# yukiteruono/pbsim3

Measured on NVIDIA B200. Metric: simulated Gbp/s, higher is better.
Workload: dtype int32

## Files before the change

### pbsim_b200/csrc/engine.cu

```cuda
#include <cuda_runtime.h>

#include <algorithm>
#include <climits>
#include <cmath>
#include <cstdarg>
#include <cstdio>
#include <cstring>
#include <cub/device/device_radix_sort.cuh>
#include <cub/device/device_scan.cuh>
#include <condition_variable>
#include <deque>
#include <mutex>
#include <string>
#include <thread>
#include <vector>

#include "../../include/pbsim_cuda.h"
#include "emit.cuh"
#include "gz_kernels.cuh"
#include "k0_genome.cuh"
#include "model_image.hpp"
#include "sample_plan.hpp"
#include "seg_kernels.cuh"
#include "sim_kernels.cuh"
// ... 571 lines not shown
  const int64_t d0 = e->run.replay_starts[s0];
  const int64_t d1 = (s0 + n_sub < e->run.replay_nsubreads) ? e->run.replay_starts[s0 + n_sub] : e->run.replay_ndraws;
  c.next_start_after = (s0 + n_sub < e->run.replay_nsubreads) ? d1 : e->run.replay_ndraws;
  if (d0 < 0 || d1 < d0 || d1 > e->run.replay_ndraws) return fail(e, PBSIM_E_REPLAY, "replay starts are not monotone");
  if (upload(e, e->d_draws, e->run.replay_draws + d0, (size_t)(d1 - d0))) return PBSIM_E_CUDA;
  if (upload(e, e->d_starts, e->run.replay_starts + s0, (size_t)n_sub)) return PBSIM_E_CUDA;
  c.A.rng.draws = e->d_draws.as<int32_t>();
  c.A.rng.draws_base = d0;
  c.A.rng.draws_end = d1;
  c.A.rng.starts = e->d_starts.as<int64_t>();
  return 0;
}

int plan(pbsim_engine *e, BatchCtx &c) {
  Batch &B = e->B;
  const uint32_t seg_min_len = c.use_segments ? (uint32_t)e->seg_min_len : 0u;
  if (c.sample)
    k_plan_sample<<<nblk(B.n_reads, 256), 256, 0, e->st>>>(c.A.G, c.Pl, *c.sb, B, e->cap_num, e->cap_den, c.spec ? 1u : 0u,
                                                             c.A.rng.seed, c.A.M.uniform_bias ? 1u : 0u, seg_min_len);
  else
    k_plan<<<nblk(B.n_reads, 256), 256, 0, e->st>>>(c.A.M, c.A.G, device_set(e), c.A.rng, B, c.clip_room, e->cap_num,
                                                      e->cap_den, c.qs ? 8u : 16u, seg_min_len, e->seg_extra,
                                                      e->chain_chunk_eff());
  e->launches++;
  return schedule_ctas(e, e->d_bins, B.key_in, B.key_out, B.idx_in, B.order, B.n_sub, 0, c.cta_threads, true, &c.cta);
}

int size_slots(pbsim_engine *e, BatchCtx &c) {
  Batch &B = e->B;
  unsigned long long *hctrl = host_ctrl(e);
  unsigned long long *tmp = u64_slice(e, kSliceScanIn);
  unsigned long long *seg_off = u64_slice(e, kSliceSegOff), *chunk_off = u64_slice(e, kSliceChunkOff);
  int rc;
  if ((rc = widen_scan(e, B.cap, B.n_sub, tmp, reinterpret_cast<unsigned long long *>(B.ev_off)))) return rc;
  if ((rc = widen_scan(e, B.ck_cap, B.n_sub, tmp, reinterpret_cast<unsigned long long *>(B.ck_off)))) return rc;
  if (c.use_segments) {
    if ((rc = widen_scan(e, B.nseg, B.n_sub, tmp, seg_off))) return rc;
    if (peek(e, hctrl + 2, seg_off + B.n_sub, 8)) return PBSIM_E_CUDA;
    if ((rc = widen_scan(e, B.nchunk, B.n_sub, tmp, chunk_off))) return rc;
    if (peek(e, hctrl + 4, chunk_off + B.n_sub, 8)) return PBSIM_E_CUDA;
  }
  if (peek(e, hctrl, B.ev_off + B.n_sub, 8)) return PBSIM_E_CUDA;
  if (peek(e, hctrl + 1, B.ck_off + B.n_sub, 8)) return PBSIM_E_CUDA;
  CK(cudaStreamSynchronize(e->st));
  c.n_seg_total = c.use_segments ? hctrl[2] : 0;
  c.n_chunk_total = c.use_segments ? hctrl[4] : 0;
  if (c.n_seg_total > 0x7FFFFFF0ull) return fail(e, PBSIM_E_INVALID, "too many segments in one batch");
  CK(e->d_ev.ensure((size_t)hctrl[0] * (c.qs ? 2 : 1) + 256));
  CK(e->d_ck.ensure((size_t)hctrl[1] * sizeof(Ckpt) + 256));
  if (c.n_seg_total > 0) CK(e->d_seg.ensure((size_t)c.n_seg_total * (6 * 4 + sizeof(SegResult)) + 256));
  return 0;
}

void pass1_sequential(pbsim_engine *e, BatchCtx &c) {
  SimArgs &A = c.A;
  set_ctas(A, c.cta);
  A.ev = e->d_ev.as<uint8_t>();
  A.ck = e->d_ck.as<Ckpt>();
  const uint32_t grid = c.cta.slots;
  if (c.sample) {
    if (c.replay) k_sim_sample<PBSIM_RNG_REPLAY><<<grid, kSimThreads, 0, e->st>>>(A, c.Pl, *c.sb, 0u);
    else k_sim_sample<PBSIM_RNG_PHILOX><<<grid, kSimThreads, 0, e->st>>>(A, c.Pl, *c.sb, 0u);
  } else if (c.qs) {
    if (c.replay) k_sim_qshmm<PBSIM_RNG_REPLAY><<<grid, kSimThreads, kQsSmemBytes, e->st>>>(A);
    else k_sim_qshmm<PBSIM_RNG_PHILOX><<<grid, kSimThreads, kQsSmemBytes, e->st>>>(A);
  } else {
    const uint32_t smem = e->er_smem_bar_off + 16;
    if (c.replay) k_sim_errhmm<PBSIM_RNG_REPLAY><<<grid, kErrThreads, smem, e->st>>>(A, e->er_smem_bar_off);
    else k_sim_errhmm<PBSIM_RNG_PHILOX><<<grid, kErrThreads, smem, e->st>>>(A, e->er_smem_bar_off);
  }
  e->launches++;
}

int pass1_segments(pbsim_engine *e, BatchCtx &c) {
  const Batch &B = e->B;
  const uint32_t nseg = (uint32_t)c.n_seg_total;
  SegBatch S;
  S.n_seg_total = nseg;
  S.seg_off = reinterpret_cast<const uint64_t *>(u64_slice(e, kSliceSegOff));
  S.seg_res = e->d_seg.as<SegResult>();
  uint32_t *u = reinterpret_cast<uint32_t *>(S.seg_res + nseg);
  uint32_t **seg_arrays[] = {&S.seg_sub, &S.seg_key_in, &S.seg_key_out, &S.seg_id_in, &S.seg_order, &S.seg_state};
  for (size_t i = 0; i < 6; ++i) *seg_arrays[i] = u + i * nseg;
  k_seg_fill<<<nblk(B.n_sub, 256), 256, 0, e->st>>>(B, S, c.pass);
  CtaSchedule sc;
  int rc = schedule_ctas(e, e->d_seg_bins, S.seg_key_in, S.seg_key_out, S.seg_id_in, S.seg_order, nseg, 20, c.cta_threads,
                         false, &sc);
  if (rc) return rc;
  SegArgs SA;
  SA.keys = c.A.keys;
  SA.M = c.A.M;
  SA.G = c.A.G;
  SA.bias_one = e->d_biasone.as<uint8_t>();
  SA.B = B;
  SA.S = S;
  set_ctas(SA, sc);
  SA.ev = e->d_ev.as<uint8_t>();
  SA.pool_q = c.Pl.quals;
  SA.pool_start = c.Pl.start;
  if (c.n_chunk_total > 0) {
    const uint32_t nch = (uint32_t)c.n_chunk_total;
    const uint32_t chain_threads = c.qs ? (uint32_t)kChainThreads : c.cta_threads;
    CK(e->d_chunk.ensure((size_t)nch * 5 * 4 + 64));
    ChunkBatch C;
    C.n_chunks = nch;
    C.per_chunk = e->chain_chunk_eff();
    C.qs = c.qs ? 1u : 0u;
    C.chunk_off = reinterpret_cast<const uint64_t *>(u64_slice(e, kSliceChunkOff));
    uint32_t **chunk_arrays[] = {&C.sub, &C.key_in, &C.key_out, &C.id_in, &C.order};
    for (size_t i = 0; i < 5; ++i) *chunk_arrays[i] = e->d_chunk.as<uint32_t>() + i * nch;
    k_chunk_fill<<<nblk(B.n_sub, 256), 256, 0, e->st>>>(B, C, c.pass);
    CtaSchedule cc;
    if ((rc = schedule_ctas(e, e->d_chunk_bins, C.key_in, C.key_out, C.id_in, C.order, nch, 0, chain_threads, true, &cc)))
      return rc;
    SegArgs CA = SA;
    set_ctas(CA, cc);
    CK(cudaEventRecord(e->ev_chain[0], e->st));
    if (c.qs) k_chain_chunk<<<cc.slots, kChainThreads, kQsSmemBytes, e->st>>>(CA, C);
    else k_chain_chunk_err<<<cc.slots, kErrThreads, e->er_smem_bar_off + 16, e->st>>>(CA, C, e->er_smem_bar_off);
    CK(cudaEventRecord(e->ev_chain[1], e->st));
    e->launches += 2;
  }
  CK(cudaEventRecord(e->ev_seg[0], e->st));
  const uint32_t end_grid = nblk((uint64_t)B.n_sub * 32, 128);
  if (c.qs) {
    if (c.sample) k_sim_seg<true><<<sc.slots, kSimThreads, 0, e->st>>>(SA);
    else k_sim_seg<false><<<sc.slots, kSimThreads, 0, e->st>>>(SA);
    CK(cudaEventRecord(e->ev_seg[1], e->st));
    k_find_end<<<end_grid, 128, 0, e->st>>>(B, S, c.A.G, SA.bias_one, c.pass, SA.ev, e->d_ck.as<Ckpt>(), c.A.M.qs_fast,
                                            c.sample ? 1u : 0u);
  } else {
    k_sim_seg_err<<<sc.slots, kErrThreads, e->er_smem_bar_off + 16, e->st>>>(SA, e->er_smem_bar_off);
    CK(cudaEventRecord(e->ev_seg[1], e->st));
    k_find_end_err<<<end_grid, 128, 0, e->st>>>(B, S, c.A.G, SA.keys, SA.bias_one, c.pass, SA.ev, e->d_ck.as<Ckpt>());
  }
  e->launches += 3;
  e->seg_batches++;
  return 0;
}

int sample_redo(pbsim_engine *e, BatchCtx &c) {
  Batch &B = e->B;
  unsigned long long *ctrl = e->d_ctrl.as<unsigned long long>(), *hctrl = host_ctrl(e);
  hctrl[6] = 0;
  CK(cudaMemsetAsync(ctrl + 6, 0, 8, e->st));
  k_sample_redo<<<nblk(B.n_reads, 256), 256, 0, e->st>>>(B, ctrl + 6);
  if (peek(e, hctrl + 6, ctrl + 6, 8)) return PBSIM_E_CUDA;
  CK(cudaStreamSynchronize(e->st));
  e->launches += 2;
  if (hctrl[6] == 0) return 0;
  const int rc =
      schedule_ctas(e, e->d_bins, B.key_in, B.key_out, B.idx_in, B.order, B.n_sub, 0, c.cta_threads, true, &c.cta);
  if (rc) return rc;
  if (c.replay) k_sim_sample<PBSIM_RNG_REPLAY><<<c.cta.slots, kSimThreads, 0, e->st>>>(c.A, c.Pl, *c.sb, 1u);
  else k_sim_sample<PBSIM_RNG_PHILOX><<<c.cta.slots, kSimThreads, 0, e->st>>>(c.A, c.Pl, *c.sb, 1u);
  e->launches++;
  e->sample_redo_groups += (int64_t)hctrl[6];
  if (hctrl[6] * 2 > c.sb->n_groups) e->sample_spec_run = false;
  return 0;
}

int quota_cut(pbsim_engine *e, BatchCtx &c, int attempt) {
  const Batch &B = e->B;
  const uint32_t n_reads = B.n_reads, n_sub = B.n_sub;
  unsigned long long *ctrl = e->d_ctrl.as<unsigned long long>(), *hctrl = host_ctrl(e);
  unsigned long long *rl0 = u64_slice(e, kSliceScanIn);
  unsigned long long *prefix = u64_slice(e, kSliceRlen0Prefix);
  k_rlen0<<<nblk(n_reads, 256), 256, 0, e->st>>>(B.rlen, n_reads, c.pass, rl0);
  const int rc = excl_scan(e, rl0, prefix, n_reads);
  if (rc) return rc;
  hctrl[0] = n_reads;
  hctrl[1] = 0;
  hctrl[2] = 0;
  hctrl[3] = 0;
  CK(cudaMemcpyAsync(ctrl, hctrl, 32, cudaMemcpyHostToDevice, e->st));
  if (c.sample)
    k_find_cut_sample<<<nblk(n_reads, 256), 256, 0, e->st>>>(prefix, n_reads, e->len_total, e->run.len_quota, ctrl);
  else if (c.clip_room < 0)
    k_find_cut<<<nblk(n_reads, 256), 256, 0, e->st>>>(prefix, B.plan_raw, n_reads, e->len_total, e->run.len_quota, ctrl);
  k_batch_totals<<<nblk(n_sub, 256), 256, 0, e->st>>>(prefix, B.rlen, B.flags, n_reads, c.pass, ctrl);
  e->launches += 3;
  if (c.replay) {
    k_check_replay<<<nblk(n_sub, 256), 256, 0, e->st>>>(c.A.rng.starts, B.draws_used, B.plan_wlen, (uint32_t)e->glen, n_sub,
                                                        c.pass, c.next_start_after, ctrl,
                                                        reinterpret_cast<unsigned int *>(&ctrl[3]));
    e->launches++;
  }
  if (peek(e, hctrl, ctrl, 32)) return PBSIM_E_CUDA;
  CK(cudaStreamSynchronize(e->st));
  const uint32_t flags = (uint32_t)hctrl[2];
  if (flags & 2u) return fail(e, PBSIM_E_PARAM, "a read drew an accuracy for which the model has no usable tables");
  float pass1_ms = 0, ms = 0;
  CK(cudaEventElapsedTime(&pass1_ms, e->ev_k[0], e->ev_k[1]));
  e->sim_ms += pass1_ms;
  if (c.n_seg_total > 0) {
    CK(cudaEventElapsedTime(&ms, e->ev_seg[0], e->ev_seg[1]));
    e->seg_ms += ms;
    if (c.n_chunk_total > 0) {
      CK(cudaEventElapsedTime(&ms, e->ev_chain[0], e->ev_chain[1]));
      e->chain_ms += ms;
    }
  }
  if (getenv("PBSIM_DEBUG"))
    fprintf(stderr, "[pbsim] batch reads=%u sub=%u segments=%llu flags=%u pass1_ms=%.2f attempt=%d\n", n_reads, n_sub,
            (unsigned long long)c.n_seg_total, flags, pass1_ms, attempt);
  return 0;
}

int emit_batch(pbsim_engine *e, const BatchCtx &c, BatchResult *out) {
  const Batch &B = e->B;
  const uint32_t nv_sub = out->n_valid_reads * c.pass;
  if (nv_sub == 0) return 0;
  unsigned long long *hctrl = host_ctrl(e);

  unsigned long long *reads_size = u64_slice(e, kSliceReadsSize);
  unsigned long long *maf_size = u64_slice(e, kSliceMafSize);
  unsigned long long *ntiles = u64_slice(e, kSliceNtiles);
  unsigned long long *reads_off = u64_slice(e, kSliceReadsOff);
  unsigned long long *maf_off = u64_slice(e, kSliceMafOff);
// ... 551 lines not shown
  if (rc != 1) return rc;
  e->held_set = it.set;
  c->first_read = it.first_read;
  c->n_reads = it.n_reads;
  c->bases = it.bases;
  c->reads_bytes = (int64_t)it.reads_bytes;
  c->maf_bytes = (int64_t)it.maf_bytes;
  c->reads_text_bytes = (int64_t)it.reads_text_bytes;
  c->maf_text_bytes = (int64_t)it.maf_text_bytes;
  c->reads = reinterpret_cast<const char *>(e->out[it.set].reads.p);
  c->maf = reinterpret_cast<const char *>(e->out[it.set].maf.p);
  c->on_device = 1;
  return 1;
}

int build_replay_read_map(pbsim_engine *e) {
  const pbsim_run &run = e->run;
  const int64_t pass = e->model.pass_num;
  const int64_t n_logged = run.replay_nsubreads / pass;
  std::vector<uint32_t> map_tr, map_k;
  map_tr.reserve((size_t)n_logged);
  map_k.reserve((size_t)n_logged);
  int64_t idx = 0;
  for (uint32_t t = 0; t < (uint32_t)e->set_n && idx < n_logged; ++t) {
    const uint32_t tlen = e->h_set_start[t + 1] - e->h_set_start[t];
    const uint32_t rank = (tlen + 999u) / 1000u;
    for (uint64_t k = 1; k <= e->h_set_nr[t] && idx < n_logged; ++k) {
      const int64_t st = run.replay_starts[idx * pass];
      if (st < 0 || st + 3 > run.replay_ndraws) return fail(e, PBSIM_E_REPLAY, "replay log exhausted while mapping the reads of the set");
      const uint32_t d0 = (uint32_t)run.replay_draws[st], d1 = (uint32_t)run.replay_draws[st + 1],
                     d2 = (uint32_t)run.replay_draws[st + 2];
      uint32_t len = (uint32_t)e->h_prob2len[d0 % (uint32_t)e->model.len_rand_value];
      const uint32_t acc = e->h_prob2acc[d1 % (uint32_t)e->model.accuracy_rand_value];
      const uint32_t index = d2 % e->h_ssp_mod[rank] + 1u;
      uint32_t ssp = 100u;
      for (uint32_t j = 0; j < 21u; ++j) {
        const uint32_t en = e->h_ssp_ends[rank * 21u + j];
        if (en == 0xFFFFu) break;
        if (index <= en) {
          ssp = j * 5u;
          break;
        }
      }
      const double value = ssp == 0u ? 0.0 : ((double)ssp - 2.5) / 100;
      volatile double prod = (double)tlen * value;
      const uint32_t offset = (uint32_t)(int)(prod + 0.5);
      if ((uint64_t)offset + len > tlen) len = offset < tlen ? tlen - offset : 0u;
      map_tr.push_back(t);
      map_k.push_back((uint32_t)k);
      ++idx;
      if (acc == 100u) k = len;
    }
  }
  if (idx != n_logged)
    return fail(e, PBSIM_E_REPLAY, "the replay log holds %lld reads but the set accounts for %lld", (long long)n_logged,
                (long long)idx);
  int rc;
  if ((rc = upload(e, e->d_map_tr, map_tr.data(), map_tr.size()))) return rc;
  if ((rc = upload(e, e->d_map_k, map_k.data(), map_k.size()))) return rc;
  CK(cudaStreamSynchronize(e->st));
  e->replay_map = true;
  e->run.max_reads = idx;
  return 0;
}

}

extern "C" {

int pbsim_cuda_abi_version(void) { return PBSIM_ABI_VERSION; }

const char *pbsim_cuda_last_error(const pbsim_engine *e) { return e ? e->err.c_str() : g_create_error.c_str(); }

int pbsim_cuda_create(pbsim_engine **out, int device) {
  pbsim_engine *e = nullptr;
  if (!out) return fail(e, PBSIM_E_INVALID, "null output pointer");
  int n = 0;
  cudaError_t ce = cudaGetDeviceCount(&n);
  if (ce != cudaSuccess || n == 0)
    return fail(e, PBSIM_E_CUDA, "no usable CUDA device (%s); libpbsim_cuda has no CPU fallback",
                ce == cudaSuccess ? "device count is 0" : cudaGetErrorString(ce));
  if (device < 0 || device >= n) return fail(e, PBSIM_E_INVALID, "device %d out of range (0..%d)", device, n - 1);
  CK(cudaSetDevice(device));
  CK(cudaFuncSetAttribute(k_chain_chunk, cudaFuncAttributePreferredSharedMemoryCarveout, cudaSharedmemCarveoutMaxShared));
  CK(cudaFuncSetAttribute(k_emit_rows<PBSIM_METHOD_QSHMM>, cudaFuncAttributePreferredSharedMemoryCarveout,
                          cudaSharedmemCarveoutMaxShared));
  CK(cudaFuncSetAttribute(k_emit_rows<PBSIM_METHOD_ERRHMM>, cudaFuncAttributePreferredSharedMemoryCarveout,
                          cudaSharedmemCarveoutMaxShared));
  CK(cudaFuncSetAttribute(k_gz_encode, cudaFuncAttributeMaxDynamicSharedMemorySize, (int)kGzEncodeSmem));
  pbsim_engine *ne = new pbsim_engine();
  ne->device = device;
  cudaError_t c1 = cudaStreamCreateWithFlags(&ne->st, cudaStreamNonBlocking);
  cudaError_t c2 = cudaStreamCreateWithFlags(&ne->st_copy, cudaStreamNonBlocking);
  cudaError_t c3 = cudaEventCreate(&ne->ev0);
  cudaError_t c4 = cudaEventCreate(&ne->ev1);
  if (c1 != cudaSuccess || c2 != cudaSuccess || c3 != cudaSuccess || c4 != cudaSuccess) {
    delete ne;
    return fail(e, PBSIM_E_CUDA, "cannot create CUDA streams/events");
  }
  cudaEventCreate(&ne->ev_copy);
  for (auto &ev : ne->ev_k) cudaEventCreate(&ev);
  for (auto &ev : ne->ev_user) cudaEventCreate(&ev);
  for (auto &ev : ne->ev_gz) cudaEventCreate(&ev);
  for (auto &ev : ne->ev_seg) cudaEventCreate(&ev);
  for (auto &ev : ne->ev_chain) cudaEventCreate(&ev);
  std::memset(&ne->model, 0, sizeof ne->model);
  std::memset(&ne->emitp, 0, sizeof ne->emitp);
  *out = ne;
  return 0;
}

void pbsim_cuda_destroy(pbsim_engine *e) {
  if (!e) return;
  cudaSetDevice(e->device);
  stop_producer(e);
  cudaStreamSynchronize(e->st_copy);
  cudaStreamSynchronize(e->st);
  cudaEventDestroy(e->ev_copy);
  for (auto &ev : e->ev_k) cudaEventDestroy(ev);
  for (auto &ev : e->ev_user) cudaEventDestroy(ev);
  for (auto &ev : e->ev_gz) cudaEventDestroy(ev);
  for (auto &ev : e->ev_seg) cudaEventDestroy(ev);
  for (auto &ev : e->ev_chain) cudaEventDestroy(ev);
  cudaEventDestroy(e->ev0);
  cudaEventDestroy(e->ev1);
  cudaStreamDestroy(e->st);
  cudaStreamDestroy(e->st_copy);
  delete e;
}

int pbsim_cuda_set_model(pbsim_engine *e, const pbsim_model *m) {
  if (!e || !m) return PBSIM_E_INVALID;
  CK(cudaSetDevice(e->device));
  const bool sample = m->method == PBSIM_METHOD_SAMPLE;
  if (m->method != PBSIM_METHOD_QSHMM && m->method != PBSIM_METHOD_ERRHMM && !sample)
    return fail(e, PBSIM_E_INVALID, "method must be qshmm, errhmm or sample");
  if (sample && m->pass_num != 1)
    return fail(e, PBSIM_E_INVALID, "sampling-based simulation supports only single-pass");
  if (!sample &&
      (m->pass_num < 1 || m->len_rand_value < 1 || m->accuracy_rand_value < 1 || !m->prob2len || !m->prob2accuracy))
    return fail(e, PBSIM_E_INVALID, "model samplers are empty");
  if (m->len_max > 1000000) return fail(e, PBSIM_E_INVALID, "length-max above FASTQ_LEN_MAX (1000000)");
  if (!e->img.build(*m)) return fail(e, PBSIM_E_INVALID, "model tables: %s", e->img.error.c_str());
  e->model = *m;
  if (sample) {
    e->h_prob2len.assign(1, 0);
    e->h_prob2acc.assign(1, 0);
    e->model.len_rand_value = e->model.accuracy_rand_value = 1;
  } else {
    e->h_prob2len.assign(m->prob2len, m->prob2len + m->len_rand_value);
    e->h_prob2acc.assign(m->prob2accuracy, m->prob2accuracy + m->accuracy_rand_value);
  }
  {
    double acc = 0;
    for (int32_t v : e->h_prob2len) acc += v;
    e->table_mean_len = acc / e->h_prob2len.size();
  }
  e->model.prob2len = e->h_prob2len.data();
  e->model.prob2accuracy = e->h_prob2acc.data();
  if (upload(e, e->d_blob, e->img.blob.data(), e->img.blob.size())) return PBSIM_E_CUDA;
  if (upload(e, e->d_acc, e->img.acc, PBSIM_NACC)) return PBSIM_E_CUDA;
  if (upload(e, e->d_prob2len, e->h_prob2len.data(), e->h_prob2len.size())) return PBSIM_E_CUDA;
  if (upload(e, e->d_prob2acc, e->h_prob2acc.data(), e->h_prob2acc.size())) return PBSIM_E_CUDA;
  CK(e->d_qs_tabs.ensure(kQsTabBytes));
  CK(e->d_qs_thr_hp.ensure(PBSIM_NQV * 48));
  CK(e->d_qs_thr_hp32.ensure(PBSIM_NQV * 48));
  CK(e->d_er_bias.ensure(std::max<size_t>(e->img.er_bias.size() * 2, 16) + 64));
// ... 437 lines not shown
```

### pbsim_b200/csrc/seg_kernels.cuh

```cuda
#pragma once
#include <cuda_runtime.h>
#include <stdint.h>

#include "sim_kernels.cuh"

namespace pb {

struct SegBatch {
  uint32_t n_seg_total;
  const uint64_t *seg_off;
  uint32_t *seg_sub;
  uint32_t *seg_key_in;
  uint32_t *seg_key_out;
  uint32_t *seg_id_in;
  uint32_t *seg_order;
  SegResult *seg_res;
  uint32_t *seg_state;
};

__global__ void k_seg_fill(Batch B, SegBatch S, uint32_t pass_num) {
  const uint32_t s = blockIdx.x * blockDim.x + threadIdx.x;
  if (s >= B.n_sub) return;
  const uint64_t lo = S.seg_off[s], hi = S.seg_off[s + 1];
  if (hi == lo) return;
  const uint32_t meta = B.plan_meta[s / pass_num];
  const uint32_t acc = meta & 0xFFu;
  for (uint64_t i = lo; i < hi; ++i) {
    S.seg_sub[i] = s;
    S.seg_key_in[i] = acc << 21;
    S.seg_id_in[i] = (uint32_t)i;
  }
}

struct ChunkBatch {
  uint32_t n_chunks, per_chunk;
  uint32_t qs;
  const uint64_t *chunk_off;
  uint32_t *sub, *key_in, *key_out, *id_in, *order;
};

__global__ void k_chunk_fill(Batch B, ChunkBatch C, uint32_t pass_num) {
  const uint32_t s = blockIdx.x * blockDim.x + threadIdx.x;
  if (s >= B.n_sub) return;
  const uint64_t lo = C.chunk_off[s], hi = C.chunk_off[s + 1];
  if (hi == lo) return;
  const uint32_t acc = B.plan_meta[s / pass_num] & 0xFFu;
  const uint32_t nseg = B.nseg[s];
  const uint32_t per = (hi - lo == 1u) ? nseg : C.per_chunk;
  for (uint64_t i = lo; i < hi; ++i) {
    const bool qs = C.qs != 0u;
    const uint32_t k_from = (uint32_t)(i - lo) * per, k_to = min(k_from + per, qs ? nseg : nseg - 1u);
    const uint32_t work = k_to - k_from + (k_from > 0u ? 1u : 0u);
    C.sub[i] = s;
    C.key_in[i] = (acc << 21) | (0xFFFFFu - min(work, 0xFFFFFu));
    C.id_in[i] = (uint32_t)i;
  }
}

struct SegArgs {
  PhiloxKeys keys;
  DeviceModel M;
  DeviceGenome G;
  const uint8_t *bias_one;
  Batch B;
  SegBatch S;
  const uint32_t *cta_order, *cta_first, *bin_lo, *bin_hi;
  uint8_t *ev;
  const uint8_t *pool_q;
  const uint64_t *pool_start;
};

constexpr int kSegWarps = kSimThreads / 32;
#ifndef PB_CHAIN_THREADS
#define PB_CHAIN_THREADS 128
#endif
constexpr int kChainThreads = PB_CHAIN_THREADS;

template <bool SAMPLE>
__global__ void __launch_bounds__(kSimThreads) k_sim_seg(SegArgs A) {
  __shared__ __align__(16) QsFast s_fast[PBSIM_NQV];
  __shared__ __align__(16) uint8_t s_freq[QsBlobLayout::freq_bytes];
  __shared__ __align__(16) uint8_t s_q[kSegWarps][PB_TILE];
  uint32_t acc, lo, hi;
  if (!cta_assignment(A.cta_order, A.cta_first, A.bin_lo, A.bin_hi, &acc, &lo, &hi)) return;
  AccEntry ae = A.M.acc[SAMPLE ? 0u : acc];
  if (SAMPLE) ae.has_model = 1;
  {
    uint32_t *d = reinterpret_cast<uint32_t *>(s_fast);
    const uint32_t *src = reinterpret_cast<const uint32_t *>(A.M.qs_fast);
    for (uint32_t i = threadIdx.x; i < PBSIM_NQV * 4u; i += blockDim.x) d[i] = src[i];
    if (!SAMPLE && !ae.has_model) {
      uint32_t *f = reinterpret_cast<uint32_t *>(s_freq);
      const uint32_t *fs = reinterpret_cast<const uint32_t *>(A.M.blob + ae.blob_off);
      for (uint32_t i = threadIdx.x; i < QsBlobLayout::freq_bytes / 4u; i += blockDim.x) f[i] = fs[i];
    }
  }
  __syncthreads();
  const uint32_t lane = threadIdx.x & 31u, warp = threadIdx.x >> 5;
  QsView T;
  T.t2 = nullptr;
  T.emis = nullptr;
  T.freq = s_freq;
  T.has_model = ae.has_model;
  T.init_mod = ae.init_mod;
  T.freq_mod = ae.freq_mod;
  T.thr = nullptr;
  T.thr_hp = nullptr;
  T.qc_prob = nullptr;
  T.thr32 = reinterpret_cast<const QsThr *>(A.M.qs_thr32);
  T.thr_hp32 = nullptr;
  T.fast = s_fast;
  for (uint32_t i = lo + warp; i < hi; i += kSegWarps) {
    const uint32_t seg = A.S.seg_order[i];
    const uint32_t s = A.S.seg_sub[seg];
    const uint32_t k = seg - (uint32_t)A.S.seg_off[s];
    const uint32_t r = s / A.M.pass_num, pass = s % A.M.pass_num;
    const uint32_t read_id = (uint32_t)(A.B.first_read + 1u + r);
    const uint32_t c1 = pass << 16;
    uint16_t *ev = reinterpret_cast<uint16_t *>(A.ev) + A.B.ev_off[s] + (uint64_t)k * PB_SEG_STRIDE;
    QsLaneTotals t;
    t.nsub = t.nins = t.ndel = t.prob = t.big = 0;
    constexpr uint32_t kIters = PB_TILE / (32u * PB_GROUP);
    uint2 q[kIters];
    if (SAMPLE) {
      const uint8_t *qp = A.pool_q + A.pool_start[A.B.plan_tr[r]];
      const uint32_t len = A.B.plan_wlen[r];
#pragma unroll
      for (uint32_t it = 0; it < kIters; ++it) {
        const uint32_t p = k * PB_TILE + lane * PB_GROUP + it * 32u * PB_GROUP;
        uint32_t b[PB_GROUP];
#pragma unroll
        for (uint32_t u = 0; u < PB_GROUP; ++u) b[u] = p + u < len ? (uint32_t)__ldg(qp + p + u) - 33u : 0u;
        q[it] = make_uint2(b[0] | (b[1] << 16), b[2] | (b[3] << 16));
      }
    } else if (ae.has_model) {
#pragma unroll
      for (uint32_t it = 0; it < kIters; ++it)
        q[it] = *reinterpret_cast<const uint2 *>(ev + lane * PB_GROUP + it * 32u * PB_GROUP);
    }
#pragma unroll
    for (uint32_t it = 0; it < kIters; ++it) {
      const uint32_t j = lane * PB_GROUP + it * 32u * PB_GROUP;
      uint32_t qv[PB_GROUP];
      if (SAMPLE || ae.has_model) {
        qv[0] = q[it].x & 0x7Fu; qv[1] = (q[it].x >> 16) & 0x7Fu; qv[2] = q[it].y & 0x7Fu; qv[3] = (q[it].y >> 16) & 0x7Fu;
      } else {
        qs_freq_qualities(T, A.keys, read_id, c1, k * PB_TILE + j, qv);
      }
      uint32_t w0, w1;
      qs_error_lane(s_fast, A.keys, read_id, c1, k * PB_TILE + j, qv, w0, w1, t);
      *reinterpret_cast<uint2 *>(ev + j) = make_uint2(w0, w1);
    }
    const uint32_t big = __any_sync(0xFFFFFFFFu, t.big != 0u) ? 1u : 0u;
    SegResult res;
    if (big) {
      __syncwarp();
      for (uint32_t j = lane; j < PB_TILE; j += 32u) s_q[warp][j] = (uint8_t)(ev[j] & 0x7Fu);
      __syncwarp();
      if (lane == 0) {
        qshmm_segment_generic(T, A.keys, read_id, pass, k * PB_TILE, k == 0, s_q[warp], ev, res);
        A.S.seg_res[seg] = res;
      }
      __syncwarp();
      continue;
    }
    const uint32_t cnt = __reduce_add_sync(0xFFFFFFFFu, t.nsub | (t.nins << 16));
    uint32_t ndel = __reduce_add_sync(0xFFFFFFFFu, t.ndel);
    const uint32_t plo = __reduce_add_sync(0xFFFFFFFFu, t.prob & 0xFFFFu);
    const uint32_t phi = __reduce_add_sync(0xFFFFFFFFu, t.prob >> 16);
    if (k == 0) {
      __syncwarp();
      if (lane == 0) ndel -= qs_fix_leading(T, A.keys, read_id, c1, ev);
    }
    if (lane == 0) {
      res.n_entries = PB_TILE;
      res.ref_adv = PB_TILE - (cnt >> 16) + ndel;
      res.nsub = cnt & 0xFFFFu;
      res.ndel = ndel;
      res.flags = 0;
      res.pad = 0;
      res.prob = (uint64_t)plo + ((uint64_t)phi << 16);
      A.S.seg_res[seg] = res;
    }
  }
}

__global__ void __launch_bounds__(kChainThreads) k_chain_chunk(SegArgs A, ChunkBatch C) {
  extern __shared__ __align__(128) uint8_t smem[];
  uint32_t acc, lo, hi;
  if (!cta_assignment(A.cta_order, A.cta_first, A.bin_lo, A.bin_hi, &acc, &lo, &hi)) return;
  const AccEntry ae = A.M.acc[acc];
  uint64_t *bar = reinterpret_cast<uint64_t *>(smem + kQsSmemBar);
  if (threadIdx.x == 0) mbar_init(bar, 1);
  __syncthreads();
  if (threadIdx.x == 0) {
    mbar_expect_tx(bar, ae.blob_bytes);
    tma_bulk_g2s(smem, A.M.blob + ae.blob_off, ae.blob_bytes, bar);
  }
  mbar_wait(bar, 0);
  const uint32_t i = lo + threadIdx.x;
  if (i >= hi) return;
  const uint32_t id = C.order[i];
  const uint32_t s = C.sub[id];
  const uint32_t c = id - (uint32_t)C.chunk_off[s];
  const uint32_t n_ch = (uint32_t)(C.chunk_off[s + 1] - C.chunk_off[s]);
  const uint32_t r = s / A.M.pass_num, pass = s % A.M.pass_num;
  const uint32_t read_id = (uint32_t)(A.B.first_read + 1u + r);
  const uint32_t nseg = A.B.nseg[s];
  const uint32_t per = n_ch == 1u ? nseg : C.per_chunk;
  const uint32_t k_from = c * per, k_to = min(k_from + per, nseg);
  QsView T;
  T.t2 = reinterpret_cast<const uint32_t *>(smem + QsBlobLayout::t2_off);
  T.emis = smem + QsBlobLayout::emis_off;
  T.freq = smem;
  T.has_model = ae.has_model;
  T.init_mod = ae.init_mod;
  T.freq_mod = ae.freq_mod;
  T.thr = nullptr;
  T.thr_hp = nullptr;
  T.qc_prob = nullptr;
  T.thr32 = nullptr;
  T.thr_hp32 = nullptr;
  T.fast = nullptr;
  uint32_t row = 0, mod = ae.init_mod, emod = 1;
  if (k_from > 0u) {
    QsSegAux X;
    X.tmod = smem + QsBlobLayout::tmod_off;
    X.emodv = smem + QsBlobLayout::emodv_off;
    X.reach = ae.reach;
    qshmm_segment_start(T, X, A.keys, read_id, pass, k_from * PB_TILE, ae.seg_ok ? ae.seg_ok : 512u, row, mod, emod);
  }
  __syncwarp();
  qshmm_quality_range(T, A.keys, read_id, pass, row, mod, emod, k_from, k_to,
                      reinterpret_cast<uint16_t *>(A.ev) + A.B.ev_off[s]);
}

__global__ void __launch_bounds__(kErrThreads) k_chain_chunk_err(SegArgs A, ChunkBatch C, uint32_t smem_bar_off) {
  extern __shared__ __align__(128) uint8_t smem[];
  uint32_t acc, lo, hi;
  if (!cta_assignment(A.cta_order, A.cta_first, A.bin_lo, A.bin_hi, &acc, &lo, &hi)) return;
  const AccEntry ae = A.M.acc[acc];
  uint64_t *bar = reinterpret_cast<uint64_t *>(smem + smem_bar_off);
  const uint32_t edel_bytes = ((ae.nstates + 1u) * 2u + 15u) / 16u * 16u;
  if (threadIdx.x == 0) mbar_init(bar, 1);
  __syncthreads();
  if (threadIdx.x == 0) {
    mbar_expect_tx(bar, ae.blob_bytes + edel_bytes);
    tma_bulk_g2s(smem, A.M.blob + ae.blob_off, ae.blob_bytes, bar);
    tma_bulk_g2s(smem + ae.blob_bytes, A.M.er_bias + ae.bias_off, edel_bytes, bar);
  }
  mbar_wait(bar, 0);
  const uint32_t i = lo + threadIdx.x;
  if (i >= hi) return;
  const uint32_t id = C.order[i];
  const uint32_t s = C.sub[id];
  const uint32_t c = id - (uint32_t)C.chunk_off[s];
  const uint32_t n_ch = (uint32_t)(C.chunk_off[s + 1] - C.chunk_off[s]);
  const uint32_t r = s / A.M.pass_num, pass = s % A.M.pass_num;
  const uint32_t read_id = (uint32_t)(A.B.first_read + 1u + r);
  const uint32_t nseg = A.B.nseg[s];
  const uint32_t per = n_ch == 1u ? nseg : C.per_chunk;
  const uint32_t k_from = c * per, k_to = min(k_from + per, nseg - 1u);
  ErView T;
  uint32_t t2o, emo, emodo;
  er_blob_bytes(ae.nstates, &t2o, &emo, &emodo);
  T.t2 = reinterpret_cast<const uint16_t *>(smem + t2o);
  T.emis = smem + emo;
  T.emod = reinterpret_cast<const uint16_t *>(smem + emodo);
  T.edel = reinterpret_cast<const uint16_t *>(smem + ae.blob_bytes);
  T.edel_hp = A.M.er_bias + ae.bias_off + (ae.nstates + 1u);
  T.init_mod = ae.init_mod;
  T.mode = ae.mode;
  T.rate_mag = ae.rate_mag;
  HpProbe hp;
  const uint32_t meta = A.B.plan_meta[r];
  hp.enabled = (meta >> 9) & 1u;
  hp.win.ascii = A.G.ascii;
  hp.win.hp4 = A.G.hp4;
  hp.win.offset = A.B.plan_off[r];
  hp.win.wlen = A.B.plan_wlen[r];
  hp.win.minus = (meta >> 8) & 1u;
  hp.xm = A.G.xm;
  hp.bias_one = A.bias_one;
  uint32_t *rec = A.S.seg_state + A.S.seg_off[s];
  uint32_t state = 0, mod = ae.init_mod;
  bool pzero = true;
  if (k_from == 0u) {
    errhmm_state_at(T, A.keys, hp, read_id, pass, k_to * PB_TILE, state, mod, pzero, rec);
    return;
  }
  errhmm_segment_start(T, T.emod + (ae.nstates + 1u), ae.reach, A.keys, hp, read_id, pass, k_from * PB_TILE,
                       ae.seg_ok ? ae.seg_ok : 512u, state, mod, pzero);
  __syncwarp();
  if (pzero) {
    errhmm_state_at(T, A.keys, hp, read_id, pass, k_to * PB_TILE, state, mod, pzero, rec);
    return;
  }
  errhmm_chain_range(T, A.keys, read_id, pass, state, mod, k_from * PB_TILE, k_to * PB_TILE, rec);
}

__global__ void __launch_bounds__(128) k_find_end(Batch B, SegBatch S, DeviceGenome G, const uint8_t *bias_one,
                                                         uint32_t pass_num, uint8_t *ev, Ckpt *ck, const QsFast *fast,
                                                         uint32_t sample) {
  const uint32_t s = (blockIdx.x * blockDim.x + threadIdx.x) >> 5;
  const uint32_t lane = threadIdx.x & 31u;
  if (s >= B.n_sub) return;
  const uint64_t lo = S.seg_off[s], hi = S.seg_off[s + 1];
  if (hi == lo) return;
  const uint32_t r = s / pass_num;
  const uint32_t meta = B.plan_meta[r];
  const uint32_t wlen = B.plan_wlen[r];
  HpProbe hp;
  hp.enabled = (meta >> 9) & 1u;
  hp.win.ascii = G.ascii;
  hp.win.hp4 = G.hp4;
  hp.win.offset = B.plan_off[r];
  hp.win.wlen = wlen;
// ... 300 lines not shown
```

### pbsim_b200/csrc/sim_core.cuh

```cuda
#pragma once
#include <math.h>
#include <stdint.h>

#if defined(__CUDACC__)
#define PB_HD __host__ __device__ __forceinline__
#define PB_HD_NOINLINE __host__ __device__ __noinline__
#else
#define PB_HD inline
#define PB_HD_NOINLINE
#endif

#define PB_TILE 1024u
#define PB_QS_ROW 100u
#define PB_ER_ROW 1000u
#define PB_KIND_MATCH 0u
#define PB_KIND_SUB 1u
#define PB_KIND_INS 2u
#define PB_KIND_DEL 3u
#define PB_QS_DEL_SAT 15u
#define PB_QS_CONT_SAT 16383u

namespace pb {

PB_HD uint32_t mulhi32(uint32_t a, uint32_t b) {
// ... 756 lines not shown
        uint32_t last_t = 0;
        for (uint64_t m = mask; m; m &= m - 1ull) {
#if defined(__CUDA_ARCH__)
          const uint32_t s = (uint32_t)__ffsll((long long)m) - 1u;
#else
          const uint32_t s = (uint32_t)__builtin_ctzll(m);
#endif
          last_t = T.t2[s * PB_QS_ROW + mulhi32(wdraw, A.tmod[s])];
          next |= 1ull << qs_state_of_row(last_t & 0xFFFFu);
        }
        mask = next;
        if ((mask & (mask - 1ull)) == 0ull) {
          single = true;
          s_row = last_t & 0xFFFFu;
          s_mod = (last_t >> 16) & 0xFFu;
          s_emod = last_t >> 24;
        }
      }
    }
    if (single) {
      row = s_row; mod = s_mod; emod = s_emod;
      return true;
    }
  }
}

PB_HD void store_u16x8(uint16_t *dst, const uint32_t v[4]) {
#if defined(__CUDA_ARCH__)
  *reinterpret_cast<uint4 *>(dst) = make_uint4(v[0], v[1], v[2], v[3]);
#else
  for (int i = 0; i < 4; ++i) { dst[2 * i] = (uint16_t)v[i]; dst[2 * i + 1] = (uint16_t)(v[i] >> 16); }
#endif
}

PB_HD void qshmm_quality_range(const QsView &T, const PhiloxKeys &K, uint32_t read_id, uint32_t pass, uint32_t row,
                               uint32_t mod, uint32_t emod, uint32_t k_from, uint32_t k_to, uint16_t *slots) {
  const uint32_t c1 = pass << 16;
  uint32_t nx[8];
  philox_block_keys(K, (k_from * PB_TILE) >> 2, c1, read_id, 2u, nx);
  philox_block_keys(K, ((k_from * PB_TILE) >> 2) + 1u, c1, read_id, 2u, nx + 4);
  for (uint32_t k = k_from; k < k_to; ++k) {
    uint16_t *slot = slots + (uint64_t)k * PB_SEG_STRIDE;
    for (uint32_t j = 0; j < PB_TILE; j += 8u) {
      const uint32_t p = k * PB_TILE + j;
      uint32_t cw[8];
#pragma unroll
      for (uint32_t u = 0; u < 8u; ++u) cw[u] = nx[u];
      philox_block_keys(K, (p >> 2) + 2u, c1, read_id, 2u, nx);
      philox_block_keys(K, (p >> 2) + 3u, c1, read_id, 2u, nx + 4);
      uint32_t out[4];
#pragma unroll
      for (uint32_t u = 0; u < 8u; ++u) {
        const uint32_t t = T.t2[row + mulhi32(cw[u] & 0xFFFF0000u, mod)];
        row = t & 0xFFFFu;
        mod = (t >> 16) & 0xFFu;
        emod = t >> 24;
        const uint32_t qv = T.emis[row + mulhi32(cw[u] << 16, emod)];
        if (u & 1u) out[u >> 1] |= qv << 16;
        else out[u >> 1] = qv;
      }
      store_u16x8(slot + j, out);
    }
  }
}

PB_HD void qs_freq_qualities(const QsView &T, const PhiloxKeys &K, uint32_t read_id, uint32_t c1, uint32_t p,
                             uint32_t qv[PB_GROUP]) {
  uint32_t q[4];
  philox_block_keys(K, p >> 2, c1, read_id, 2u, q);
#pragma unroll
  for (uint32_t u = 0; u < PB_GROUP; ++u) qv[u] = T.freq[mulhi32(q[u], T.freq_mod)];
}

struct QsLaneTotals {
  uint32_t nsub, nins, ndel, prob, big;
};
PB_HD uint32_t pb_popc(uint32_t x) {
#if defined(__CUDA_ARCH__)
  return (uint32_t)__popc(x);
#else
  return (uint32_t)__builtin_popcount(x);
#endif
}
PB_HD void qs_error_lane(const QsFast *fast, const PhiloxKeys &K, uint32_t read_id, uint32_t c1, uint32_t p,
                         const uint32_t qv[PB_GROUP], uint32_t &w0, uint32_t &w1, QsLaneTotals &t) {
  uint32_t x[PB_GROUP], y[PB_GROUP], e[PB_GROUP];
  error_words(K, read_id, c1, p, x, y);
#pragma unroll
  for (uint32_t u = 0; u < PB_GROUP; ++u) {
    const QsFast th = fast[qv[u]];
    uint32_t nd;
    const uint32_t base = qs_event(th, qv[u], x[u], y[u], nd);
    t.prob += th.prob;
    t.big |= nd >= PB_QS_DEL_SAT ? 1u : 0u;
    e[u] = base | ((nd < PB_QS_DEL_SAT ? nd : PB_QS_DEL_SAT) << 12);
  }
  w0 = e[0] | (e[1] << 16);
  w1 = e[2] | (e[3] << 16);
  t.nsub += pb_popc((w0 & 0x00800080u) | ((w1 & 0x00800080u) << 1));
  t.nins += pb_popc((w0 & 0x01000100u) | ((w1 & 0x01000100u) << 1));
  const uint32_t dd = ((w0 >> 12) & 0x000F000Fu) + ((w1 >> 12) & 0x000F000Fu);
  t.ndel += (dd & 0xFFFFu) + (dd >> 16);
}

PB_HD uint32_t qs_fix_leading(const QsView &T, const PhiloxKeys &K, uint32_t read_id, uint32_t c1, uint16_t *ev) {
  uint32_t removed = 0;
  for (uint32_t p = 0; p < PB_TILE; ++p) {
    const uint32_t v = ev[p];
    if (((v >> 7) & 3u) != PB_KIND_INS) break;
    uint32_t x, y;
    error_words_at(K, read_id, c1, p, x, y);
    if (y < T.thr32[v & 0x7Fu].del0) break;
    removed += v >> 12;
    ev[p] = (uint16_t)(v & 0x0FFFu);
  }
  return removed;
}

PB_HD void qshmm_segment_generic(const QsView &T, const PhiloxKeys &K, uint32_t read_id, uint32_t pass,
                                 uint32_t p_start, bool first_segment, const uint8_t *qv_in, uint16_t *ev,
                                 SegResult &res) {
  uint32_t R = first_segment ? 0u : 1u;
  uint32_t radv = 0, n = 0, nsub = 0, ndel = 0;
  uint64_t prob = 0;
  const uint32_t c1 = pass << 16;
  res.flags = 0;
  for (uint32_t j = 0; j < PB_TILE; ++j) {
    if (n + 2u * PB_GROUP > PB_SEG_STRIDE) { res.flags |= 1u; break; }
    const uint32_t P = p_start + j;
    uint32_t qv;
    if (T.has_model) {
      qv = qv_in[j];
    } else {
      uint32_t q[4];
      philox_block_keys(K, P >> 2, c1, read_id, 2u, q);
      const uint32_t k4 = P & 3u;
      qv = T.freq[mulhi32(k4 == 0u ? q[0] : (k4 == 1u ? q[1] : (k4 == 2u ? q[2] : q[3])), T.freq_mod)];
    }
    uint32_t x, y;
    error_words_at(K, read_id, c1, P, x, y);
    const QsFast th = T.fast[qv];
    prob += th.prob;
    const bool is_sub = x < th.sub;
    const bool is_err = x < th.ins;
    const uint32_t info = is_sub ? (((x & 0xFFFu) * 3u) >> 12) : (is_err ? (y & 7u) : 0u);
    const uint32_t kind = is_sub ? PB_KIND_SUB : (is_err ? PB_KIND_INS : PB_KIND_MATCH);
    nsub += is_sub ? 1u : 0u;
    const uint32_t a = (is_err && !is_sub) ? 0u : 1u;
    R += a;
    radv += a;
    uint32_t nd = 0;
    if (y < (R != 0u ? th.del : T.thr32[qv].del0)) {
      nd = 1;
      for (uint32_t d = del_next(y); nd < (1u << 20) && d < th.del; d = del_next(d)) ++nd;
      R += nd;
      radv += nd;
    }
    ndel += nd;
    const uint32_t base = qv | (kind << 7) | (info << 9);
    if (nd < PB_QS_DEL_SAT) {
      ev[n++] = (uint16_t)(base | (nd << 12));
    } else {
      ev[n++] = (uint16_t)(base | (PB_QS_DEL_SAT << 12));
      uint32_t rest = nd - PB_QS_DEL_SAT;
      for (;;) {
        if (n + 2u * PB_GROUP > PB_SEG_STRIDE) { res.flags |= 1u; break; }
        const uint32_t c = rest < PB_QS_CONT_SAT ? rest : PB_QS_CONT_SAT;
        ev[n++] = (uint16_t)((c & 0x7Fu) | (3u << 7) | ((c >> 7) << 9));
        if (c < PB_QS_CONT_SAT) break;
        rest -= PB_QS_CONT_SAT;
      }
      if (res.flags) break;
    }
  }
  while (n & (PB_GROUP - 1u)) ev[n++] = (uint16_t)PB_QS_PAD;
  res.n_entries = n;
  res.ref_adv = radv;
  res.nsub = nsub;
  res.ndel = ndel;
  res.pad = 0;
  res.prob = prob;
}

PB_HD void qshmm_error_segment(const QsView &T, const PhiloxKeys &K, uint32_t read_id, uint32_t pass, uint32_t p_start,
                               bool first_segment, uint16_t *ev, SegResult &res) {
  const uint32_t c1 = pass << 16;
  QsLaneTotals t;
  t.nsub = t.nins = t.ndel = t.prob = t.big = 0;
  uint64_t prob = 0;
  uint8_t qsave[PB_TILE];
  for (uint32_t j = 0; j < PB_TILE; j += PB_GROUP) {
    uint32_t qv[PB_GROUP], e[PB_GROUP];
    if (T.has_model) {
#pragma unroll
      for (uint32_t u = 0; u < PB_GROUP; ++u) qv[u] = ev[j + u] & 0x7Fu;
    } else {
      qs_freq_qualities(T, K, read_id, c1, p_start + j, qv);
    }
#pragma unroll
    for (uint32_t u = 0; u < PB_GROUP; ++u) qsave[j + u] = (uint8_t)qv[u];
    t.prob = 0;
    uint32_t w0, w1;
    qs_error_lane(T.fast, K, read_id, c1, p_start + j, qv, w0, w1, t);
    e[0] = w0 & 0xFFFFu; e[1] = w0 >> 16; e[2] = w1 & 0xFFFFu; e[3] = w1 >> 16;
    prob += t.prob;
#pragma unroll
    for (uint32_t u = 0; u < PB_GROUP; ++u) ev[j + u] = (uint16_t)e[u];
  }
  if (t.big) {
    qshmm_segment_generic(T, K, read_id, pass, p_start, first_segment, qsave, ev, res);
    return;
  }
  if (first_segment) t.ndel -= qs_fix_leading(T, K, read_id, c1, ev);
  res.n_entries = PB_TILE;
  res.ref_adv = PB_TILE - t.nins + t.ndel;
  res.nsub = t.nsub;
  res.ndel = t.ndel;
  res.flags = 0;
  res.pad = 0;
  res.prob = prob;
}

struct HpProbe {
  uint32_t enabled;
  WindowRef win;
  const uint32_t *xm;
  const uint8_t *bias_one;
  PB_HD bool suppress(uint32_t r_prev) const {
    const uint32_t g = win.gidx(r_prev);
    const uint32_t blk = g >> 10;
    if (((xm[blk >> 5] >> (blk & 31u)) & 1u) == 0u) return false;
    return bias_one[win.hp(r_prev)] == 0;
  }
};

struct TileWalk {
  uint32_t n_entries, positions, ref_adv, nsub, ndel;
  uint32_t ended;
  uint64_t prob;
};

PB_HD TileWalk qshmm_walk_tile(uint16_t *ev, uint32_t n_entries, uint32_t R_start, uint32_t wlen,
                               const QsFast *fast, const HpProbe &hp, uint32_t *blocked_io = nullptr,
                               uint32_t p_left = 0xFFFFFFFFu) {
  TileWalk t;
  t.n_entries = 0; t.positions = 0; t.ref_adv = 0; t.nsub = 0; t.ndel = 0; t.ended = 0; t.prob = 0;
  uint32_t R = R_start;
  bool blocked = blocked_io ? (*blocked_io != 0u) : false;
  for (uint32_t i = 0; i < n_entries; ++i) {
    const uint32_t v = ev[i];
    const uint32_t kind = (v >> 7) & 3u;
    const bool cont = kind == 3u;
    const uint32_t part = cont ? ((v & 0x7Fu) | ((v >> 9) << 7)) : (v >> 12);
    bool last_position = false;
    if (!cont) {
      if (R >= wlen || t.positions >= p_left) { t.ended = 1; break; }
      t.prob += fast[v & 0x7Fu].prob;
      t.positions += 1u;
      t.nsub += (kind == PB_KIND_SUB) ? 1u : 0u;
      R += (kind == PB_KIND_INS) ? 0u : 1u;
      blocked = false;
      if (t.positions == p_left) blocked = last_position = true;
    }
    uint32_t take = 0;
    if (!blocked) {
      const uint32_t room = wlen - R;
      uint32_t lim = part < room ? part : room;
      if (hp.enabled) {
        for (uint32_t j = 0; j < lim; ++j) {
          if (R + j != 0u && hp.suppress(R + j - 1u)) { lim = j; break; }
        }
      }
      take = lim;
      if (take < part) blocked = true;
    }
    if (take != part) {
      if (cont) ev[i] = (uint16_t)((take & 0x7Fu) | (3u << 7) | ((take >> 7) << 9));
      else ev[i] = (uint16_t)((v & 0x0FFFu) | (take << 12));
    }
    t.ndel += take;
    R += take;
    t.n_entries = i + 1u;
    if (R >= wlen || last_position) { t.ended = 1; break; }
  }
  t.ref_adv = R - R_start;
  if (blocked_io) *blocked_io = blocked ? 1u : 0u;
  return t;
}

struct SegRead {
  uint32_t n_tiles, rlen, ncol, nsub, nins, ndel, flags;
  double accuracy;
};

PB_HD uint32_t qshmm_segments_for(uint32_t wlen, float rho) {
  const double need = (double)wlen * (double)rho * 1.015 + 8.0 * sqrt((double)wlen) + 64.0;
  return (uint32_t)((need + (double)(PB_TILE - 1u)) / (double)PB_TILE);
}

PB_HD void qshmm_finish_segmented(uint16_t *ev_base, const SegResult *seg, uint32_t n_seg, uint32_t wlen,
                                  const QsFast *fast, const HpProbe &hp, Ckpt *ck, SegRead &out,
                                  uint32_t p_len = 0xFFFFFFFFu) {
  uint32_t R = 0, P = 0, D = 0, nsub = 0;
// ... 412 lines not shown
```

Measured before the change: 114.3.

## Fuse QS chain quality generation with error simulation in pass-1 kernel

The chained QSHMM chunk kernel now generates qualities and error events for each tile in one pass, writing segment results directly. The separate k_sim_seg launch and its CTA scheduling are skipped for chained subreads in non-sample QS mode, unless some accuracy entry is frequency-only. The aim is to remove a second pass over the event buffer, a re-read of the qualities, and a scheduling sort. The cost is a heavier chain kernel that serialises more per-thread work, and fast threshold tables are now loaded into shared memory by TMA.

```diff
diff --git a/pbsim_b200/csrc/engine.cu b/pbsim_b200/csrc/engine.cu
--- a/pbsim_b200/csrc/engine.cu
+++ b/pbsim_b200/csrc/engine.cu
@@ -677,11 +677,15 @@
   uint32_t *u = reinterpret_cast<uint32_t *>(S.seg_res + nseg);
   uint32_t **seg_arrays[] = {&S.seg_sub, &S.seg_key_in, &S.seg_key_out, &S.seg_id_in, &S.seg_order, &S.seg_state};
   for (size_t i = 0; i < 6; ++i) *seg_arrays[i] = u + i * nseg;
-  k_seg_fill<<<nblk(B.n_sub, 256), 256, 0, e->st>>>(B, S, c.pass);
-  CtaSchedule sc;
-  int rc = schedule_ctas(e, e->d_seg_bins, S.seg_key_in, S.seg_key_out, S.seg_id_in, S.seg_order, nseg, 20, c.cta_threads,
-                         false, &sc);
-  if (rc) return rc;
+  bool freq_only = false;
+  for (const AccEntry &a : e->img.acc) freq_only |= a.valid && !a.has_model;
+  const bool seg_pass = !c.qs || c.sample || freq_only;
+  k_seg_fill<<<nblk(B.n_sub, 256), 256, 0, e->st>>>(B, S, c.pass, c.qs && !c.sample ? 1u : 0u);
+  CtaSchedule sc = {};
+  int rc = 0;
+  if (seg_pass && (rc = schedule_ctas(e, e->d_seg_bins, S.seg_key_in, S.seg_key_out, S.seg_id_in, S.seg_order, nseg, 20,
+                                      c.cta_threads, false, &sc)))
+    return rc;
   SegArgs SA;
   SA.keys = c.A.keys;
   SA.M = c.A.M;
@@ -711,7 +715,7 @@
     SegArgs CA = SA;
     set_ctas(CA, cc);
     CK(cudaEventRecord(e->ev_chain[0], e->st));
-    if (c.qs) k_chain_chunk<<<cc.slots, kChainThreads, kQsSmemBytes, e->st>>>(CA, C);
+    if (c.qs) k_qs_pass1<<<cc.slots, kChainThreads, kQsSmemBytes, e->st>>>(CA, C);
     else k_chain_chunk_err<<<cc.slots, kErrThreads, e->er_smem_bar_off + 16, e->st>>>(CA, C, e->er_smem_bar_off);
     CK(cudaEventRecord(e->ev_chain[1], e->st));
     e->launches += 2;
@@ -720,7 +724,8 @@
   const uint32_t end_grid = nblk((uint64_t)B.n_sub * 32, 128);
   if (c.qs) {
     if (c.sample) k_sim_seg<true><<<sc.slots, kSimThreads, 0, e->st>>>(SA);
-    else k_sim_seg<false><<<sc.slots, kSimThreads, 0, e->st>>>(SA);
+    else if (seg_pass) k_sim_seg<false><<<sc.slots, kSimThreads, 0, e->st>>>(SA);
+    e->launches += seg_pass ? 1 : 0;
     CK(cudaEventRecord(e->ev_seg[1], e->st));
     k_find_end<<<end_grid, 128, 0, e->st>>>(B, S, c.A.G, SA.bias_one, c.pass, SA.ev, e->d_ck.as<Ckpt>(), c.A.M.qs_fast,
                                             c.sample ? 1u : 0u);
@@ -728,8 +733,9 @@
     k_sim_seg_err<<<sc.slots, kErrThreads, e->er_smem_bar_off + 16, e->st>>>(SA, e->er_smem_bar_off);
     CK(cudaEventRecord(e->ev_seg[1], e->st));
     k_find_end_err<<<end_grid, 128, 0, e->st>>>(B, S, c.A.G, SA.keys, SA.bias_one, c.pass, SA.ev, e->d_ck.as<Ckpt>());
-  }
-  e->launches += 3;
+    e->launches++;
+  }
+  e->launches += 2;
   e->seg_batches++;
   return 0;
 }
@@ -1447,7 +1453,7 @@
                 ce == cudaSuccess ? "device count is 0" : cudaGetErrorString(ce));
   if (device < 0 || device >= n) return fail(e, PBSIM_E_INVALID, "device %d out of range (0..%d)", device, n - 1);
   CK(cudaSetDevice(device));
-  CK(cudaFuncSetAttribute(k_chain_chunk, cudaFuncAttributePreferredSharedMemoryCarveout, cudaSharedmemCarveoutMaxShared));
+  CK(cudaFuncSetAttribute(k_qs_pass1, cudaFuncAttributePreferredSharedMemoryCarveout, cudaSharedmemCarveoutMaxShared));
   CK(cudaFuncSetAttribute(k_emit_rows<PBSIM_METHOD_QSHMM>, cudaFuncAttributePreferredSharedMemoryCarveout,
                           cudaSharedmemCarveoutMaxShared));
   CK(cudaFuncSetAttribute(k_emit_rows<PBSIM_METHOD_ERRHMM>, cudaFuncAttributePreferredSharedMemoryCarveout,
diff --git a/pbsim_b200/csrc/seg_kernels.cuh b/pbsim_b200/csrc/seg_kernels.cuh
--- a/pbsim_b200/csrc/seg_kernels.cuh
+++ b/pbsim_b200/csrc/seg_kernels.cuh
@@ -18,16 +18,17 @@
   uint32_t *seg_state;
 };
 
-__global__ void k_seg_fill(Batch B, SegBatch S, uint32_t pass_num) {
+__global__ void k_seg_fill(Batch B, SegBatch S, uint32_t pass_num, uint32_t skip_chained) {
   const uint32_t s = blockIdx.x * blockDim.x + threadIdx.x;
   if (s >= B.n_sub) return;
   const uint64_t lo = S.seg_off[s], hi = S.seg_off[s + 1];
   if (hi == lo) return;
   const uint32_t meta = B.plan_meta[s / pass_num];
   const uint32_t acc = meta & 0xFFu;
+  const bool skip = skip_chained != 0u && B.nchunk[s] != 0u;
   for (uint64_t i = lo; i < hi; ++i) {
     S.seg_sub[i] = s;
-    S.seg_key_in[i] = acc << 21;
+    S.seg_key_in[i] = skip ? ((uint32_t)kBins << 20) : acc << 21;
     S.seg_id_in[i] = (uint32_t)i;
   }
 }
@@ -133,16 +134,12 @@
         for (uint32_t u = 0; u < PB_GROUP; ++u) b[u] = p + u < len ? (uint32_t)__ldg(qp + p + u) - 33u : 0u;
         q[it] = make_uint2(b[0] | (b[1] << 16), b[2] | (b[3] << 16));
       }
-    } else if (ae.has_model) {
-#pragma unroll
-      for (uint32_t it = 0; it < kIters; ++it)
-        q[it] = *reinterpret_cast<const uint2 *>(ev + lane * PB_GROUP + it * 32u * PB_GROUP);
     }
 #pragma unroll
     for (uint32_t it = 0; it < kIters; ++it) {
       const uint32_t j = lane * PB_GROUP + it * 32u * PB_GROUP;
       uint32_t qv[PB_GROUP];
-      if (SAMPLE || ae.has_model) {
+      if (SAMPLE) {
         qv[0] = q[it].x & 0x7Fu; qv[1] = (q[it].x >> 16) & 0x7Fu; qv[2] = q[it].y & 0x7Fu; qv[3] = (q[it].y >> 16) & 0x7Fu;
       } else {
         qs_freq_qualities(T, A.keys, read_id, c1, k * PB_TILE + j, qv);
@@ -185,7 +182,7 @@
   }
 }
 
-__global__ void __launch_bounds__(kChainThreads) k_chain_chunk(SegArgs A, ChunkBatch C) {
+__global__ void __launch_bounds__(kChainThreads) k_qs_pass1(SegArgs A, ChunkBatch C) {
   extern __shared__ __align__(128) uint8_t smem[];
   uint32_t acc, lo, hi;
   if (!cta_assignment(A.cta_order, A.cta_first, A.bin_lo, A.bin_hi, &acc, &lo, &hi)) return;
@@ -194,8 +191,9 @@
   if (threadIdx.x == 0) mbar_init(bar, 1);
   __syncthreads();
   if (threadIdx.x == 0) {
-    mbar_expect_tx(bar, ae.blob_bytes);
+    mbar_expect_tx(bar, ae.blob_bytes + PBSIM_NQV * 16u);
     tma_bulk_g2s(smem, A.M.blob + ae.blob_off, ae.blob_bytes, bar);
+    tma_bulk_g2s(smem + kQsSmemFast, A.M.qs_fast, PBSIM_NQV * 16u, bar);
   }
   mbar_wait(bar, 0);
   const uint32_t i = lo + threadIdx.x;
@@ -219,9 +217,9 @@
   T.thr = nullptr;
   T.thr_hp = nullptr;
   T.qc_prob = nullptr;
-  T.thr32 = nullptr;
+  T.thr32 = reinterpret_cast<const QsThr *>(A.M.qs_thr32);
   T.thr_hp32 = nullptr;
-  T.fast = nullptr;
+  T.fast = reinterpret_cast<const QsFast *>(smem + kQsSmemFast);
   uint32_t row = 0, mod = ae.init_mod, emod = 1;
   if (k_from > 0u) {
     QsSegAux X;
@@ -231,8 +229,8 @@
     qshmm_segment_start(T, X, A.keys, read_id, pass, k_from * PB_TILE, ae.seg_ok ? ae.seg_ok : 512u, row, mod, emod);
   }
   __syncwarp();
-  qshmm_quality_range(T, A.keys, read_id, pass, row, mod, emod, k_from, k_to,
-                      reinterpret_cast<uint16_t *>(A.ev) + A.B.ev_off[s]);
+  qshmm_chunk_pass1(T, A.keys, read_id, pass, row, mod, k_from, k_to, reinterpret_cast<uint16_t *>(A.ev) + A.B.ev_off[s],
+                    A.S.seg_res + A.S.seg_off[s]);
 }
 
 __global__ void __launch_bounds__(kErrThreads) k_chain_chunk_err(SegArgs A, ChunkBatch C, uint32_t smem_bar_off) {
diff --git a/pbsim_b200/csrc/sim_core.cuh b/pbsim_b200/csrc/sim_core.cuh
--- a/pbsim_b200/csrc/sim_core.cuh
+++ b/pbsim_b200/csrc/sim_core.cuh
@@ -862,10 +862,9 @@
   return (uint32_t)__builtin_popcount(x);
 #endif
 }
-PB_HD void qs_error_lane(const QsFast *fast, const PhiloxKeys &K, uint32_t read_id, uint32_t c1, uint32_t p,
-                         const uint32_t qv[PB_GROUP], uint32_t &w0, uint32_t &w1, QsLaneTotals &t) {
-  uint32_t x[PB_GROUP], y[PB_GROUP], e[PB_GROUP];
-  error_words(K, read_id, c1, p, x, y);
+PB_HD void qs_error_group(const QsFast *fast, const uint32_t qv[PB_GROUP], const uint32_t x[PB_GROUP],
+                          const uint32_t y[PB_GROUP], uint32_t &w0, uint32_t &w1, QsLaneTotals &t) {
+  uint32_t e[PB_GROUP];
 #pragma unroll
   for (uint32_t u = 0; u < PB_GROUP; ++u) {
     const QsFast th = fast[qv[u]];
@@ -881,6 +880,12 @@
   t.nins += pb_popc((w0 & 0x01000100u) | ((w1 & 0x01000100u) << 1));
   const uint32_t dd = ((w0 >> 12) & 0x000F000Fu) + ((w1 >> 12) & 0x000F000Fu);
   t.ndel += (dd & 0xFFFFu) + (dd >> 16);
+}
+PB_HD void qs_error_lane(const QsFast *fast, const PhiloxKeys &K, uint32_t read_id, uint32_t c1, uint32_t p,
+                         const uint32_t qv[PB_GROUP], uint32_t &w0, uint32_t &w1, QsLaneTotals &t) {
+  uint32_t x[PB_GROUP], y[PB_GROUP];
+  error_words(K, read_id, c1, p, x, y);
+  qs_error_group(fast, qv, x, y, w0, w1, t);
 }
 
 PB_HD uint32_t qs_fix_leading(const QsView &T, const PhiloxKeys &K, uint32_t read_id, uint32_t c1, uint16_t *ev) {
@@ -999,6 +1004,58 @@
   res.flags = 0;
   res.pad = 0;
   res.prob = prob;
+}
+
+PB_HD void qshmm_chunk_pass1(const QsView &T, const PhiloxKeys &K, uint32_t read_id, uint32_t pass, uint32_t row,
+                             uint32_t mod, uint32_t k_from, uint32_t k_to, uint16_t *slots, SegResult *res) {
+  const uint32_t c1 = pass << 16;
+  uint32_t nx[8];
+  philox_block_keys(K, (k_from * PB_TILE) >> 2, c1, read_id, 2u, nx);
+  philox_block_keys(K, ((k_from * PB_TILE) >> 2) + 1u, c1, read_id, 2u, nx + 4);
+  for (uint32_t k = k_from; k < k_to; ++k) {
+    uint16_t *slot = slots + (uint64_t)k * PB_SEG_STRIDE;
+    QsLaneTotals t;
+    t.nsub = t.nins = t.ndel = t.prob = t.big = 0;
+    uint64_t prob = 0;
+    for (uint32_t j = 0; j < PB_TILE; j += 8u) {
+      const uint32_t p = k * PB_TILE + j;
+      uint32_t cw[8], x[8], y[8], qv[8], w[4];
+#pragma unroll
+      for (uint32_t u = 0; u < 8u; ++u) cw[u] = nx[u];
+      philox_block_keys(K, (p >> 2) + 2u, c1, read_id, 2u, nx);
+      philox_block_keys(K, (p >> 2) + 3u, c1, read_id, 2u, nx + 4);
+      error_words(K, read_id, c1, p, x, y);
+      error_words(K, read_id, c1, p + 4u, x + 4, y + 4);
+#pragma unroll
+      for (uint32_t u = 0; u < 8u; ++u) {
+        const uint32_t e = T.t2[row + mulhi32(cw[u] & 0xFFFF0000u, mod)];
+        row = e & 0xFFFFu;
+        mod = (e >> 16) & 0xFFu;
+        qv[u] = T.emis[row + mulhi32(cw[u] << 16, e >> 24)];
+      }
+      t.prob = 0;
+      qs_error_group(T.fast, qv, x, y, w[0], w[1], t);
+      qs_error_group(T.fast, qv + 4, x + 4, y + 4, w[2], w[3], t);
+      prob += t.prob;
+      store_u16x8(slot + j, w);
+    }
+    if (t.big) {
+      uint8_t q[PB_TILE];
+      for (uint32_t j = 0; j < PB_TILE; ++j) q[j] = (uint8_t)(slot[j] & 0x7Fu);
+      qshmm_segment_generic(T, K, read_id, pass, k * PB_TILE, k == 0, q, slot, res[k]);
+      continue;
+    }
+    if (k == 0) t.ndel -= qs_fix_leading(T, K, read_id, c1, slot);
+    SegResult r;
+    r.n_entries = PB_TILE;
+    r.ref_adv = PB_TILE - t.nins + t.ndel;
+    r.nsub = t.nsub;
+    r.ndel = t.ndel;
+    r.flags = 0;
+    r.pad = 0;
+    r.prob = prob;
+    res[k] = r;
+  }
 }
 
 struct HpProbe {
```

Result: faster. 132.7 (median of 6 runs) (+16.0%).
